# Derek-TH-Wang/quadruped_ctrl

Hardware: AMD Instinct MI355X
Metric: convex-MPC QP solves/sec (horizon=10, 4-leg) (higher is better)
Workload: dtype f64

## Files before the change

quadruped_ctrl_amd/csrc/qmpc_kernels.hip:

```cpp
#include <hip/hip_runtime.h>
#include <stdint.h>

#include <type_traits>

#include "qmpc_device.h"
#include "qmpc_cmd.h"
#include "qmpc_wave.h"

namespace {

__device__ __forceinline__ void fmac16_rowbcast(double (&a)[16], double c, double u) {
  asm volatile(
      "s_nop 1\n\t"
      "v_fmac_f64_dpp %0, %16, %17 row_newbcast:0 row_mask:0xf bank_mask:0xf\n\t"
      "v_fmac_f64_dpp %1, %16, %17 row_newbcast:1 row_mask:0xf bank_mask:0xf\n\t"
      "v_fmac_f64_dpp %2, %16, %17 row_newbcast:2 row_mask:0xf bank_mask:0xf\n\t"
      "v_fmac_f64_dpp %3, %16, %17 row_newbcast:3 row_mask:0xf bank_mask:0xf\n\t"
      "v_fmac_f64_dpp %4, %16, %17 row_newbcast:4 row_mask:0xf bank_mask:0xf\n\t"
      "v_fmac_f64_dpp %5, %16, %17 row_newbcast:5 row_mask:0xf bank_mask:0xf\n\t"
      "v_fmac_f64_dpp %6, %16, %17 row_newbcast:6 row_mask:0xf bank_mask:0xf\n\t"
      "v_fmac_f64_dpp %7, %16, %17 row_newbcast:7 row_mask:0xf bank_mask:0xf\n\t"
      "v_fmac_f64_dpp %8, %16, %17 row_newbcast:8 row_mask:0xf bank_mask:0xf\n\t"
      "v_fmac_f64_dpp %9, %16, %17 row_newbcast:9 row_mask:0xf bank_mask:0xf\n\t"
      "v_fmac_f64_dpp %10, %16, %17 row_newbcast:10 row_mask:0xf bank_mask:0xf\n\t"
// ... 175 lines not shown
    set0 = (unsigned)__builtin_amdgcn_readlane((int)m, k0);
    const unsigned long long ne = ~(__ballot(m == set0 && lane < h) >> k0);
    run = ne ? __builtin_ctzll(ne) : 64;
    run = run < h - k0 ? run : h - k0;
  }
  const int k = (lane < 3) ? lane : (lane < 6 ? lane - 3 : 0);
  const bool rot = lane < 3, row = lane < 6;
  const float* q = P.q + (size_t)i * 4;
  const float* tr = P.traj + (size_t)i * 12 * h;
  const float T = (float)h * (float)P.dt;
  const float qw = q[0], qx = q[1], qy = q[2], qz = q[3];
  const float ang = (k == 0) ? 2.f * (qw * qx + qy * qz) : (k == 1 ? 2.f * (qw * qy - qz * qx) : P.yaw[i]);
  const float x0 = rot ? ang : P.p[(size_t)i * 3 + k];
  const float xd = rot ? P.w[(size_t)i * 3 + k] : P.v[(size_t)i * 3 + k];
  const float e = (x0 - tr[(rot ? 0 : 3) + k]) + T * (xd - tr[(rot ? 6 : 9) + k]);
  const float wk = P.weights[(size_t)i * P.weights_stride + (rot ? 0 : 3) + k];
  const float ialpha = 1.f / (P.alpha[(size_t)i * P.alpha_stride] + 1e-30f);
  const float t_acc = wk * __builtin_fabsf(e), t_dem = __builtin_sqrtf(wk * ialpha) * __builtin_fabsf(e);
  float acc = 0.f, wsum = 1e-30f, dem = 0.f;
#pragma unroll
  for (int l = 0; l < 6; ++l) {
    acc += __builtin_bit_cast(float, __builtin_amdgcn_readlane(__builtin_bit_cast(int, t_acc), l));
    wsum += __builtin_bit_cast(float, __builtin_amdgcn_readlane(__builtin_bit_cast(int, wk), l));
    dem += __builtin_bit_cast(float, __builtin_amdgcn_readlane(__builtin_bit_cast(int, t_dem), l));
  }
  float score = acc / wsum * (float)first3;
  const float demand = dem * (float)first3 / ((float)P.mass * __builtin_fabsf((float)P.gravity) + 1e-30f);
  float pattern = 0.f;
  if (set0 != 0u) {
    float c3[3] = {0.f, 0.f, 0.f};
#pragma unroll
    for (int ax = 0; ax < 3; ++ax)
#pragma unroll
      for (int f = 0; f < 4; ++f) {
        const float rv = __builtin_bit_cast(float, __builtin_amdgcn_readlane(__builtin_bit_cast(int, rraw), 4 * ax + f));
        c3[ax] += ((set0 >> f) & 1u) ? rv : 0.f;
      }
    const float inv = 1.f / (float)__builtin_popcount(set0);
    const float cx = c3[0] * inv, cy = c3[1] * inv, cz = __builtin_fabsf(c3[2] * inv);
    const float sat = __builtin_sqrtf(cx * cx + cy * cy) * (float)P.mu_inv / (cz > 1e-3f ? cz : 1e-3f);
    const float sa = sat > 0.6f ? (sat < 1.f ? sat : 1.f) : 0.f;
    const float pat = (float)run * sa - 1.5f;
    pattern = pat > 0.f ? pat : 0.f;
    score += 0.15f * pattern;
  }
  return {nst, score, demand, pattern};
}
__device__ __forceinline__ int qmpc_score_level(const float score, const float per, const int levels) {
  int b = (score > 0.f) ? (int)(per * (__log2f(score) + 6.f)) : 0;
  b = b < 0 ? 0 : (b > levels - 1 ? levels - 1 : b);
  return levels - 1 - b;
}

template <int RB>
struct Cfg {
  static constexpr bool C1 = (RB == 1 || RB == 6);
  static constexpr int NP = (RB == 4) ? 96 : (RB == 6 ? 64 : 64 * RB);
  static constexpr int CW = NP / 4;
  static constexpr int NT = 4 * NP;
  static constexpr bool BALANCE = (RB == 4);
  static constexpr int NT_LAUNCH = BALANCE ? 512 : NT;
  static constexpr int RE = (NP + 63) / 64;
  static constexpr int KMAX = C1 ? 64 : 96;
  static constexpr int KW = (KMAX + 63) / 64;
  static constexpr int NS = KMAX * (KMAX + 1) / 2;
  static constexpr int NH = NP * (NP + 1) / 2;
  static constexpr int POOL = (RB == 1) ? 2688 : (RB == 6 ? 1536 : (RB == 2 ? 11400 : (RB == 4 ? 5120 : 1176)));
  static constexpr int NPOOL = POOL;
  static constexpr int KS = C1 ? 32 : (RB == 3 ? 128 : 64);
  static constexpr bool EVENT_ENGINE = true;
  static constexpr bool GLOBAL_EVENTS = (RB == 3);
  static constexpr int KEV_GLOBAL = (RB == 3) ? 160 : 96;
  static constexpr int NHELP = C1 ? 0 : 3;
  static constexpr bool PAIRED = (RB == 2 || RB == 3);
  static constexpr int HELP_MIN_TRIPS = 3;
  static constexpr int HMAX = (RB == 3) ? 36 : 16;
  static constexpr int MIN_WAVES = (RB == 1 || RB == 4) ? 4 : (RB == 6 ? 5 : (RB == 2 ? 2 : 3));
  static constexpr int MIN_WAVES_A = (RB == 2) ? 4 : MIN_WAVES;
};

template <int RB>
struct Smem {
  using C = Cfg<RB>;
  QmpcParams par;
  static constexpr int SLOTS = (RB == 3) ? 144 : 64;
  double fmaxk[SLOTS];
  unsigned char sidx[SLOTS];
  unsigned char kslot[4 * C::HMAX];
  int nst, status;
  int mode;
  int evslot;
  int qnext;
  int prio_rank;
  int bal_simd[8], bal_cu, bal_bit;
  struct Help {
    int cmd;
    int pj1, pj2, neva, nevd, glob;
    double pa1, pa2;
    unsigned long long gptr;
  } hd;
  union U {
    struct AW {
      struct Asm {
        double Mb[4][9];
        double Nb[4][9];
        double W[12];
        static constexpr int TAB = (C::HMAX + 1) * (C::HMAX + 1);
        double ct0[TAB], ct4[TAB];
        double ct1[TAB], ct5[TAB], ct8[TAB];
        double E00[144], E11[144];
        double e[C::HMAX * 12];
        double s[3][C::HMAX * 12];
      } a;
      struct Swp {
        alignas(16) double colbuf[2][2][C::NP + 2];
        double ubuf[2][2][C::NP];
        double g[C::NP];
        double part[4][C::NP];
      } w;
    } aw;
    struct Slv {
      double Hp[C::NH];
      double Sinv[C::NPOOL];
      double D[C::NP];
    } b;
  } u;
};

#ifndef QMPC_DBG_ITER
#define QMPC_DBG_ITER 0
#endif
#define QMPC_TICK1(k)                                                \
  do {                                                               \
    if (dbg_clk && tid == 0 && iters == 0) dbg_clk[(k)] = clock64(); \
  } while (0)
#define QMPC_TICK(k)                                   \
  do {                                                 \
    if (dbg_clk && tid == 0) dbg_clk[(k)] = clock64(); \
  } while (0)

#ifdef QMPC_SWEEP_STAMP
#define QMPC_STEP_TICK(k, dep)                                                                            \
  do {                                                                                                    \
    if (PK.dbg_clk && tid == 0 && k0 == QMPC_SWEEP_STAMP) {                         \
      double dep__ = (dep);                                                                               \
      asm volatile("" ::"v"(dep__));                                                                      \
      PK.dbg_clk[(size_t)(rid + PK.batch) * 16 + (k)] = clock64();                                    \
    }                                                                                                     \
  } while (0)
#else
#define QMPC_STEP_TICK(k, dep) do { } while (0)
#endif

#ifdef QMPC_STOP_AFTER
template <int RB, int NV>
__device__ __forceinline__ void qmpc_census_dump(Smem<RB>& S, const QmpcParams& PK, int rid, int tid, const double (&regs)[NV]) {
  double acc = 0.0;
#pragma unroll
  for (int k = 0; k < NV; ++k) acc += regs[k];
  const volatile double* lds = reinterpret_cast<const volatile double*>(&S);
  for (int k = tid; k < (int)(sizeof(Smem<RB>) / 8); k += Cfg<RB>::NT) acc += lds[k];
  PK.grf[(size_t)rid * 12 + (tid % 12)] = (float)acc;
  if (tid == 0) {
    PK.status[rid] = 0;
    if (PK.iters) PK.iters[rid] = 0;
  }
}
#define QMPC_STOP(k, regs)                                  \
  do {                                                      \
    if constexpr (QMPC_STOP_AFTER == (k)) {                 \
      __syncthreads();                                      \
      qmpc_census_dump<RB>(S, PK, rid, tid, regs);          \
      __syncthreads();                                      \
      return false;                                         \
    }                                                       \
  } while (0)
#else
#define QMPC_STOP(k, regs) do { } while (0)
#endif

template <int RB, bool V5, bool CMD, bool ADMM = false, bool WARM = false, bool PHA = false, bool BIG = false, bool PRIO = false>
__device__ __forceinline__ bool solve_one(const int rid, const int tid, Smem<RB>& S, const QmpcParams& PK) {
  using C = Cfg<RB>;
  constexpr int NP = C::NP, CW = C::CW, NT = C::NT, KMAX = C::KMAX, KW = C::KW, RE = C::RE;
  const QmpcParams& P = S.par;
  const int lane = tid & (WAVE - 1);
  const int i = tid % NP;
  const int c = tid / NP;
  const int h = PK.horizon;
  const int nfs = 4 * h;
  constexpr int HMAX = C::HMAX;
  constexpr int NFG = (4 * HMAX + 63) / 64;
  long long* dbg_clk = PK.dbg_clk ? PK.dbg_clk + (size_t)rid * 16 : nullptr;
  QMPC_TICK(0);
  {
    const double none[1] = {0.0};
    (void)none;
    QMPC_STOP(-1, none);
  }
  __builtin_amdgcn_s_setprio(3);
  bool hard = false;
  int hfloor = 0;
  if (PK.hint_hard > 0) {
    const int32_t* grp = (const int32_t*)__builtin_assume_aligned(PK.hint_iters + (rid & ~15), 64);
    int mine = 0, ge = 0;
#pragma unroll
    for (int k = 0; k < 16; ++k) mine = ((rid & 15) == k) ? grp[k] : mine;
#pragma unroll
    for (int k = 0; k < 16; ++k) ge += (grp[k] >= mine) ? 1 : 0;
    mine = __builtin_amdgcn_readfirstlane(mine);
    ge = __builtin_amdgcn_readfirstlane(ge);
    const int top = __builtin_amdgcn_readfirstlane(*PK.hint_max_r);
    hard = mine >= PK.hint_hard && 5 * mine >= 3 * top && ge <= 2;
    hfloor = hard ? 3 : ((mine >= PK.hint_hard && 5 * mine >= 2 * top && ge <= 4) ? 2 : 0);
  }

  unsigned long long prio_mine = 0ull;
  unsigned long long* prio_word = nullptr;
  auto& Aa = S.u.aw.a;
  auto& Sw = S.u.aw.w;
  const int eidx0 = (tid + NT / 2) % NT;
  const bool e_thr = eidx0 < 12 * h;
  const int ek = eidx0 / 12, erow = eidx0 - 12 * ek;
  const int mt = tid % 36, mb = mt / 9, ml = (mt % 9) / 3, max_ = mt % 3;
  const int hs = h + 1, hh = hs * hs;
  constexpr bool cmdm = CMD;
  static_assert(sizeof(QmpcParams) % 4 == 0 && sizeof(QmpcParams) / 4 <= 256, "parameter block copy");
  uint32_t g_par = 0;
  if (tid < (int)(sizeof(QmpcParams) / 4)) g_par = reinterpret_cast<const uint32_t*>(&PK)[tid];
  float g_yaw = cmdm ? PK.c_rpy[(size_t)rid * 3 + 2] : PK.yaw[rid];
  float g_xdrag = cmdm ? PK.c_xci[rid] : PK.x_drag[(size_t)rid * PK.x_drag_stride];
  float c_p0 = 0.f, c_p1 = 0.f, c_p2 = 0.f;
  QmpcTrajGen tg;
  if (cmdm) {
    const float* pos = PK.c_position + (size_t)rid * 3;
    c_p0 = pos[0];
    c_p1 = pos[1];
    c_p2 = pos[2];
    const bool stand = PK.c_gait_type && PK.c_gait_type[rid] == 4;
    float vw0, vw1;
    qmpc_cmd_vdes_world(PK.c_r_body + (size_t)rid * 9, PK.c_vel_des[(size_t)rid * 3 + 0], PK.c_vel_des[(size_t)rid * 3 + 1],
                        PK.c_omni_mode, vw0, vw1);
    qmpc_cmd_traj_gen(tg, stand, stand ? PK.c_stand_traj + (size_t)rid * 6 : nullptr,
                      PK.c_rp_des ? PK.c_rp_des + (size_t)rid * 2 : nullptr, PK.c_rpy_comp + (size_t)rid * 2,
                      PK.c_yaw_des_true[rid], PK.c_wpd[(size_t)rid * 2 + 0], PK.c_wpd[(size_t)rid * 2 + 1], c_p0, c_p1,
                      PK.c_body_height, PK.c_vel_des[(size_t)rid * 3 + 2], vw0, vw1, (float)PK.dt);
  }
  auto gait_at = [&](int fs) __attribute__((always_inline)) {
    if (cmdm) {
      const int leg = fs & 3;
      return (unsigned char)qmpc_cmd_gait_bit(fs >> 2, PK.c_gait_iteration[rid], PK.c_gait_offsets[(size_t)rid * 4 + leg],
                                              PK.c_gait_durations[(size_t)rid * 4 + leg], h);
    }
    return (unsigned char)PK.gait[(size_t)rid * nfs + fs];
  };
  unsigned char g_gait = 0;
  unsigned char g_gaitx[NFG > 1 ? NFG - 1 : 1] = {};
  if (tid < nfs) g_gait = gait_at(tid);
  if constexpr (NFG > 1) {
    if (tid < WAVE) {
#pragma unroll
      for (int g = 1; g < NFG; ++g)
        if (tid + 64 * g < nfs) g_gaitx[g - 1] = gait_at(tid + 64 * g);
    }
  }
  float g_r0 = 0.f, g_r1 = 0.f, g_r2 = 0.f;
  if (tid < 72) {
    if (cmdm) {
      const float* pf = PK.c_p_foot + (size_t)rid * 12 + 3 * mb;
      g_r0 = qmpc_cmd_foot_offset(pf[0], c_p0);
      g_r1 = qmpc_cmd_foot_offset(pf[1], c_p1);
      g_r2 = qmpc_cmd_foot_offset(pf[2], c_p2);
    } else {
      const float* r = PK.r + (size_t)rid * 12;
      g_r0 = r[0 * 4 + mb];
      g_r1 = r[1 * 4 + mb];
      g_r2 = r[2 * 4 + mb];
    }
  }
  float g_q[4] = {1.f, 0.f, 0.f, 0.f}, g_w[3] = {0.f, 0.f, 0.f}, g_v[3] = {0.f, 0.f, 0.f};
  float g_p = 0.f, g_traj = 0.f, g_wt = 0.f;
  if (e_thr) {
    const float* q = (cmdm ? PK.c_orientation : PK.q) + (size_t)rid * 4;
    const float* om = (cmdm ? PK.c_omega_world : PK.w) + (size_t)rid * 3;
    const float* v = (cmdm ? PK.c_v_world : PK.v) + (size_t)rid * 3;
#pragma unroll
    for (int k = 0; k < 4; ++k) g_q[k] = q[k];
#pragma unroll
    for (int k = 0; k < 3; ++k) {
      g_w[k] = om[k];
      g_v[k] = v[k];
    }
    if (cmdm) {
      if (erow >= 3 && erow < 6) g_p = (erow == 3) ? c_p0 : (erow == 4 ? c_p1 : c_p2);
      g_traj = qmpc_cmd_traj_value(tg, ek, erow);
      g_wt = qmpc_cmd_weight(erow);
    } else {
      if (erow >= 3 && erow < 6) g_p = PK.p[(size_t)rid * 3 + (erow - 3)];
      g_traj = PK.traj[(size_t)rid * 12 * h + eidx0];
      g_wt = PK.weights[(size_t)rid * PK.weights_stride + erow];
    }
  }
  float g_w12 = 0.f;
  if (tid >= 96 && tid < 96 + 12)
    g_w12 = cmdm ? qmpc_cmd_weight(tid - 96) : PK.weights[(size_t)rid * PK.weights_stride + (tid - 96)];
  float g_alpha = cmdm ? 4e-5f : PK.alpha[(size_t)rid * PK.alpha_stride];
  double g_ct0 = 0.0, g_ct4 = 0.0, g_ct1 = 0.0, g_ct5 = 0.0, g_ct8 = 0.0;
  constexpr bool TAB2 = (HMAX + 1) * (HMAX + 1) > NT;
  double g2_ct0 = 0.0, g2_ct4 = 0.0, g2_ct1 = 0.0, g2_ct5 = 0.0, g2_ct8 = 0.0;
  if constexpr (TAB2) {
    if (tid + NT < hh) {
      g2_ct0 = PK.ctab[tid + NT];
      g2_ct4 = PK.ctab[4 * hh + tid + NT];
      g2_ct1 = PK.ctab[1 * hh + tid + NT];
      g2_ct5 = PK.ctab[5 * hh + tid + NT];
      g2_ct8 = PK.ctab[8 * hh + tid + NT];
    }
  }
  if (tid < hh) {
    g_ct0 = PK.ctab[tid];
    g_ct4 = PK.ctab[4 * hh + tid];
    g_ct1 = PK.ctab[1 * hh + tid];
    g_ct5 = PK.ctab[5 * hh + tid];
    g_ct8 = PK.ctab[8 * hh + tid];
  }
  if constexpr (PRIO && !CMD && !ADMM && !BIG && !PHA) {
    if (PK.prio_cu && (tid >> 6) == 1) {
      const QmpcKeys kk = qmpc_robot_keys_wave(PK, rid, lane);
      if (tid == 127) {
        unsigned hwid, xcc;
        asm volatile("s_getreg_b32 %0, hwreg(HW_REG_HW_ID)" : "=s"(hwid));
        asm volatile("s_getreg_b32 %0, hwreg(HW_REG_XCC_ID)" : "=s"(xcc));
        prio_word = PK.prio_cu + (((xcc & 7u) << 8) | ((hwid >> 8) & 0xffu));
        if (kk.demand >= 12.f || kk.pattern > 0.5f) {
          const int pb = qmpc_score_level(kk.score, 6.f, 64);
          prio_mine = ((unsigned long long)PK.prio_tag << 32) | ((unsigned long long)(63 - pb) << 24) | (unsigned)(rid & 0xffffff);
          __hip_atomic_fetch_max(prio_word, prio_mine, __ATOMIC_RELAXED, __HIP_MEMORY_SCOPE_AGENT);
        }
      }
    }
  }
  {
    int gg = g_gait;
    asm volatile("" : "+v"(g_par), "+v"(g_yaw), "+v"(g_xdrag), "+v"(g_alpha), "+v"(gg), "+v"(g_r0), "+v"(g_r1),
                 "+v"(g_r2), "+v"(g_q[0]), "+v"(g_q[1]), "+v"(g_q[2]), "+v"(g_q[3]), "+v"(g_w[0]), "+v"(g_w[1]),
                 "+v"(g_w[2]), "+v"(g_v[0]), "+v"(g_v[1]), "+v"(g_v[2]), "+v"(g_p), "+v"(g_traj), "+v"(g_wt),
                 "+v"(g_w12), "+v"(g_ct0), "+v"(g_ct4), "+v"(g_ct1), "+v"(g_ct5), "+v"(g_ct8));
    g_gait = (unsigned char)gg;
    if constexpr (TAB2) asm volatile("" : "+v"(g2_ct0), "+v"(g2_ct4), "+v"(g2_ct1), "+v"(g2_ct5), "+v"(g2_ct8));
  }
  if (tid < (int)(sizeof(QmpcParams) / 4)) reinterpret_cast<uint32_t*>(&S.par)[tid] = g_par;
  const double x_drag = (double)g_xdrag;
  const bool drag = (x_drag != 0.0);

  if (dbg_clk && tid == 0) {
    float sink = g_yaw + g_traj + (float)g_gait + (float)g_ct0;
    asm volatile("" ::"v"(sink));
    dbg_clk[11] = clock64();
  }
  if (tid < WAVE) {
    int base = 0;
#pragma unroll
    for (int g = 0; g < NFG; ++g) {
      const int fs = tid + 64 * g;
      const float fm = (float)(g == 0 ? g_gait : g_gaitx[g > 0 ? g - 1 : 0]) * (float)PK.f_max;
      const bool st = fs < nfs && (((ADMM || BIG) && PK.admm_mode == 1) ? true : !(fm < 0.01f && fm > -.01f));
      const unsigned long long mask = __ballot(st);
      const int pos = base + __popcll(mask & ((1ull << tid) - 1ull));
      if (st && pos < Smem<RB>::SLOTS) {
        S.sidx[pos] = (unsigned char)fs;
        S.fmaxk[pos] = (double)fm;
      }
      if (fs < 4 * HMAX) S.kslot[fs] = (st && pos < Smem<RB>::SLOTS) ? (unsigned char)pos : (unsigned char)0xff;
      base += __popcll(mask);
    }
    if (tid == 0) {
      S.nst = base;
      S.status = 0;
    }
  }
  if (PK.soln)
    for (int k = tid; k < 12 * h; k += NT) PK.soln[(size_t)rid * 12 * h + k] = 0.0;

  const double inv_m = PK.inv_mass;
  {
    float syf, cyf;
    sincosf(g_yaw, &syf, &cyf);
    const double cy = cyf, sy = syf;
    if (PK.dbg_aux && tid == 0) {
      PK.dbg_aux[(size_t)rid * 8 + 0] = cy;
      PK.dbg_aux[(size_t)rid * 8 + 1] = sy;
    }
    if (tid < 72) {
      const int b = mb, l = ml, ax = max_;
      const double ix = PK.inv_ibody[0], iy = PK.inv_ibody[1], iz = PK.inv_ibody[2];
      const double en = __builtin_fma(cy, cy, sy * sy) - 1.0;
      const double isc = 1.0 - 2.0 * en + 3.0 * en * en;
      const double I00 = (cy * cy * ix + sy * sy * iy) * isc, I01 = (cy * sy * (ix - iy)) * isc,
                   I11 = (sy * sy * ix + cy * cy * iy) * isc;
      const double rx = g_r0, ry = g_r1, rz = g_r2;
      const double cm0 = (ax == 0) ? 0.0 : (ax == 1 ? -rz : ry);
      const double cm1 = (ax == 0) ? rz : (ax == 1 ? 0.0 : -rx);
      const double cm2 = (ax == 0) ? -ry : (ax == 1 ? rx : 0.0);
      const double m0 = I00 * cm0 + I01 * cm1;
      const double m1 = I01 * cm0 + I11 * cm1;
      const double m2 = iz * cm2;
      if (tid < 36) {
        Aa.Mb[b][3 * l + ax] = (l == 0) ? m0 : (l == 1 ? m1 : m2);
      } else {
        Aa.Nb[b][3 * l + ax] = (l == 0) ? (cy * m0 + sy * m1) : (l == 1 ? (-sy * m0 + cy * m1) : m2);
      }
    } else if (tid >= 96 && tid < 96 + 12) {
      Aa.W[tid - 96] = (double)g_w12;
    }
    if (e_thr) {
      const int row = erow;
      const double t = (double)(ek + 1) * PK.dt;
      double val;
      if (row < 3) {
#pragma clang fp contract(off)
        const float w = g_q[0], x = g_q[1], y = g_q[2], z = g_q[3];
        const float a_num = (row == 0) ? 2.f * (y * z + w * x) : 2.f * (x * y + w * z);
        const float a_den = (row == 0) ? (w * w - x * x - y * y + z * z) : (w * w + x * x - y * y - z * z);
        float ang = atan2f(a_num, a_den);
        if (row == 1) {
          double asd = -2. * (double)(x * z - w * y);
          if (!(asd < .99999)) asd = .99999;
          ang = asinf((float)asd);
        }
        const double o0 = g_w[0], o1 = g_w[1], o2 = g_w[2];
        const double rate = (row == 0) ? (cy * o0 + sy * o1) : (row == 1 ? (-sy * o0 + cy * o1) : o2);
        if (PK.dbg_aux && ek == 0) PK.dbg_aux[(size_t)rid * 8 + 2 + row] = (double)ang;
        val = (double)ang + rate * t;
      } else if (row < 6) {
        val = (double)g_p + (double)(row == 3 ? g_v[0] : (row == 4 ? g_v[1] : g_v[2])) * t;
        if (row == 5) {
          val += (PK.model == 1) ? 0.5 * PK.gravity * (t * t - t * PK.dt)
                                 : 0.5 * (PK.gravity + x_drag * (double)g_v[0]) * t * t;
        }
      } else if (row < 9) {
        val = (double)(row == 6 ? g_w[0] : (row == 7 ? g_w[1] : g_w[2]));
      } else {
        val = (double)(row == 9 ? g_v[0] : (row == 10 ? g_v[1] : g_v[2]));
        if (row == 11) val += (PK.gravity + x_drag * (double)g_v[0]) * t;
      }
      Aa.e[eidx0] = (double)g_wt * (val - (double)g_traj);
    }
    if (tid < hh) {
      Aa.ct0[tid] = g_ct0;
      Aa.ct4[tid] = g_ct4;
      if (drag) {
        Aa.ct1[tid] = g_ct1;
        Aa.ct5[tid] = g_ct5;
        Aa.ct8[tid] = g_ct8;
      }
    }
    if constexpr (TAB2) {
      if (tid + NT < hh) {
        Aa.ct0[tid + NT] = g2_ct0;
        Aa.ct4[tid + NT] = g2_ct4;
        if (drag) {
          Aa.ct1[tid + NT] = g2_ct1;
          Aa.ct5[tid + NT] = g2_ct5;
          Aa.ct8[tid + NT] = g2_ct8;
        }
      }
    }
  }
  if (dbg_clk && tid == 0) dbg_clk[12] = clock64();
  __syncthreads();
  QMPC_TICK(1);
  if constexpr (PRIO && !CMD && !ADMM && !BIG && !PHA) {
    if (PK.prio_cu && tid == 127) {
      const unsigned long long pv = __hip_atomic_load(prio_word, __ATOMIC_RELAXED, __HIP_MEMORY_SCOPE_AGENT);
      S.prio_rank = (prio_mine != 0ull && pv == prio_mine) ? 0 : ((unsigned)(pv >> 32) == PK.prio_tag ? 1 : 2);
    }
  }
  {
    const double keep0[2] = {(double)g_alpha, x_drag};
    (void)keep0;
    QMPC_STOP(0, keep0);
  }
  if (PK.hint_hard > 0 && !hard) __builtin_amdgcn_s_setprio(2);
  const int nst = S.nst;
  const int n = 3 * nst;
  auto cmd_finish_state = [&]() __attribute__((always_inline)) {
    const float* pos = P.c_position + (size_t)rid * 3;
    if (!(P.c_gait_type && P.c_gait_type[rid] == 4)) {
      P.c_wpd[(size_t)rid * 2 + 0] = qmpc_cmd_clamp(P.c_wpd[(size_t)rid * 2 + 0], pos[0]);
      P.c_wpd[(size_t)rid * 2 + 1] = qmpc_cmd_clamp(P.c_wpd[(size_t)rid * 2 + 1], pos[1]);
    }
    P.c_xci[rid] = qmpc_cmd_xci_next(P.c_xci[rid], pos[2], P.c_body_height, (float)P.dt, P.c_v_world[(size_t)rid * 3 + 0]);
  };
  auto cmd_finish_forces = [&](const float* fb, int l12) __attribute__((always_inline)) {
    const int leg = l12 / 3, ii = l12 - 3 * leg;
    P.f_ff[(size_t)rid * 12 + l12] =
        qmpc_cmd_f2b(P.c_r_body + (size_t)rid * 9 + 3 * ii, fb[3 * leg], fb[3 * leg + 1], fb[3 * leg + 2]);
  };
  static_assert(!BIG || (RB == 3 && PHA && !ADMM && !WARM), "large-problem producer: an instantiation of the 192-row class");
  if (nst == 0 || n > (BIG ? 3 * Smem<RB>::SLOTS : NP)) {
    if (nst == 0) {
      if (tid < 12) P.grf[(size_t)rid * 12 + tid] = 0.f;
      if (cmdm && P.f_ff && tid < 12) P.f_ff[(size_t)rid * 12 + tid] = 0.f;
      if (tid == 0) {
        P.status[rid] = 0;
        if (P.iters) P.iters[rid] = 0;
        if (cmdm) cmd_finish_state();
      }
      if (WARM && P.ws && tid < QMPC_WS_STRIDE) P.ws[(size_t)rid * QMPC_WS_STRIDE + tid] = -1;
    } else if (P.next_list) {
      if (tid == 0) {
        const int slot = atomicAdd(P.next_count, 1);
        if (slot < P.batch) {
          P.next_list[slot] = rid;
        } else {
          P.status[rid] = QMPC_DEV_ST_WS_FULL;
          if (P.iters) P.iters[rid] = 0;
          for (int k = 0; k < 12; ++k) P.grf[(size_t)rid * 12 + k] = 0.f;
        }
      }
    } else {
      if (tid < 12) P.grf[(size_t)rid * 12 + tid] = 0.f;
      if (cmdm && P.f_ff && tid < 12) P.f_ff[(size_t)rid * 12 + tid] = 0.f;
      if (tid == 0) {
        P.status[rid] = QMPC_DEV_ST_WS_FULL;
        if (P.iters) P.iters[rid] = 0;
        if (cmdm) cmd_finish_state();
      }
    }
    __syncthreads();
    return false;
  }
  const double alpha = (double)g_alpha;
  if constexpr (PHA) {
    if (tid == 0) S.evslot = P.wk_base + atomicAdd(P.wk_count, 1);
  }
  if (tid < 144) {
    const int u = tid / 12, v = tid - 12 * u;
    const int bu = u / 3, au = u - 3 * bu, bv = v / 3, av = v - 3 * bv;
    double e00 = 0.0, e11 = 0.0;
#pragma unroll
    for (int l = 0; l < 3; ++l) {
      e00 += Aa.W[6 + l] * (Aa.Mb[bu][3 * l + au] * Aa.Mb[bv][3 * l + av]);
      e11 += Aa.W[l] * (Aa.Nb[bu][3 * l + au] * Aa.Nb[bv][3 * l + av]);
    }
    if (au == av) {
      e00 += Aa.W[9 + au] * (inv_m * inv_m);
      e11 += Aa.W[3 + au] * (inv_m * inv_m);
      if (drag && au == 0) e11 += Aa.W[11] * ((x_drag * inv_m) * (x_drag * inv_m));
    }
    Aa.E00[tid] = e00;
    Aa.E11[tid] = e11;
  }
  if constexpr (HMAX <= 16) {
    if (tid >= 64 && tid < 256) {
      const int row = (tid - 64) >> 4, st = tid & 15;
      auto shl = [](double x, auto nc) __attribute__((always_inline)) {
        constexpr int N = decltype(nc)::value;
        const unsigned long long b = (unsigned long long)__double_as_longlong(x);
        const unsigned lo = (unsigned)__builtin_amdgcn_mov_dpp((int)(unsigned)b, 0x100 + N, 0xf, 0xf, true);
        const unsigned hi = (unsigned)__builtin_amdgcn_mov_dpp((int)(unsigned)(b >> 32), 0x100 + N, 0xf, 0xf, true);
        return __longlong_as_double((long long)(((unsigned long long)hi << 32) | lo));
      };
      auto suffix = [&](double x) __attribute__((always_inline)) {
        x += shl(x, std::integral_constant<int, 1>{});
        x += shl(x, std::integral_constant<int, 2>{});
        x += shl(x, std::integral_constant<int, 4>{});
        x += shl(x, std::integral_constant<int, 8>{});
        return x;
      };
      const double e = (st < h) ? Aa.e[st * 12 + row] : 0.0;
      const double S0 = suffix(e);
      const double S1 = suffix(shl(S0, std::integral_constant<int, 1>{}));
      const double T2 = suffix(shl(S1, std::integral_constant<int, 1>{}));
      const double S2 = 2.0 * T2 + S1;
      const double dt1 = P.dt, dt2 = dt1 * dt1, dt3 = dt2 * dt1;
      if (st < h) {
        Aa.s[0][st * 12 + row] = dt1 * S0;
        Aa.s[1][st * 12 + row] = (P.model == 1) ? dt2 * S1 : dt2 * S1 + (0.5 * dt2) * S0;
        Aa.s[2][st * 12 + row] = (0.5 * dt3) * (S2 + S1) + (dt3 / 6.0) * S0;
      }
    }
  } else if (tid >= 192 && tid < 204) {
    const int row = tid - 192;
    double ek[HMAX];
#pragma unroll
    for (int k = 0; k < HMAX; ++k) ek[k] = Aa.e[(k < h ? k : 0) * 12 + row];
    const double dt1 = P.dt, dt2 = dt1 * dt1, dt3 = dt2 * dt1;
    double S0 = 0.0, S1 = 0.0, S2 = 0.0;
#pragma unroll
    for (int st = HMAX - 1; st >= 0; --st) {
      if (st < h) {
        S2 = S2 + 2.0 * S1 + S0;
        S1 = S1 + S0;
        S0 = S0 + ek[st];
        Aa.s[0][st * 12 + row] = dt1 * S0;
        Aa.s[1][st * 12 + row] = (P.model == 1) ? dt2 * S1 : dt2 * S1 + (0.5 * dt2) * S0;
        Aa.s[2][st * 12 + row] = (0.5 * dt3) * (S2 + S1) + (dt3 / 6.0) * S0;
      }
    }
  }
  __syncthreads();
  QMPC_TICK(2);
  if constexpr (PRIO && !CMD && !ADMM && !BIG && !PHA) {
    if (PK.prio_cu && __builtin_amdgcn_readfirstlane(S.prio_rank) == 1) __builtin_amdgcn_s_setprio(2);
  }
  {
    const double keep1[2] = {alpha, x_drag};
    (void)keep1;
    QMPC_STOP(1, keep1);
  }
  if constexpr (PHA) {
    if (S.evslot - P.wk_base >= P.wk_cap) {
      if (tid < 12) P.grf[(size_t)rid * 12 + tid] = 0.f;
      if (cmdm && P.f_ff && tid < 12) P.f_ff[(size_t)rid * 12 + tid] = 0.f;
      if (tid == 0) {
        P.status[rid] = QMPC_DEV_ST_WS_FULL;
        if (P.iters) P.iters[rid] = 0;
        if (cmdm) cmd_finish_state();
      }
      __syncthreads();
      return false;
    }
  }

#ifdef QMPC_BIG_STAMP
#define QMPC_BIG_TICK(k) do { if (dbg_clk && tid == 0) dbg_clk[(k)] = clock64(); } while (0)
#define QMPC_BIG_STEP_TICK(k) do { if (dbg_clk && tid == 0 && k0 == NB * QMPC_BIG_STAMP) dbg_clk[(k)] = clock64(); } while (0)
#else
#define QMPC_BIG_TICK(k) do { } while (0)
#define QMPC_BIG_STEP_TICK(k) do { } while (0)
#endif
  if constexpr (BIG) {
    constexpr int LDB = QMPC_BIG_LD, NB = 16, PD = NB + 1, NMAX = 3 * Smem<RB>::SLOTS;
    const int item = S.evslot;
    GlobalF64* const A = (GlobalF64*)P.wk_hinv + (size_t)item * ((size_t)LDB * LDB);
    auto ldA = [&](int r, int cidx) __attribute__((always_inline)) {
      return __hip_atomic_load(A + (size_t)r * LDB + cidx, __ATOMIC_RELAXED, __HIP_MEMORY_SCOPE_WORKGROUP);
    };
    const int wv = tid >> 6;
    constexpr int NWV = NT / 64;
    const double dm2 = x_drag * inv_m * inv_m;

    QMPC_BIG_TICK(8);
    double gmine = 0.0;
    if (tid < n) {
      const int ki = S.sidx[tid / 3], ax = tid % 3;
      const int st = ki >> 2, b = ki & 3;
      const double* s0 = &Aa.s[0][st * 12];
      const double* s1 = &Aa.s[1][st * 12];
      double acc = s0[9 + ax] * inv_m + s1[3 + ax] * inv_m;
#pragma unroll
      for (int l = 0; l < 3; ++l) acc += Aa.Mb[b][3 * l + ax] * s0[6 + l] + Aa.Nb[b][3 * l + ax] * s1[l];
      if (drag && ax == 0) acc += (x_drag * inv_m) * (s1[11] + Aa.s[2][st * 12 + 5]);
      gmine = 2.0 * acc;
    }
    {
      const double w11 = Aa.W[11] * dm2, w5 = Aa.W[5] * dm2, w5x = Aa.W[5] * (x_drag * dm2);
      for (int r = wv; r < n; r += NWV) {
        const int ki = S.sidx[r / 3], ai = r % 3, si = ki >> 2, u = 3 * (ki & 3) + ai;
        for (int j = lane; j < n; j += 64) {
          const int kj = S.sidx[j / 3], cax = j % 3, sj = kj >> 2;
          const int cidx = si * hs + sj, tidx = sj * hs + si, eidx = u * 12 + 3 * (kj & 3) + cax;
          double v = Aa.ct0[cidx] * Aa.E00[eidx] + Aa.ct4[cidx] * Aa.E11[eidx];
          if (drag) {
            double add = 0.0;
            if (ai == 2 && cax == 0) add = Aa.ct1[cidx] * w11 + Aa.ct5[cidx] * w5;
            if (ai == 0 && cax == 2) add = Aa.ct1[tidx] * w11 + Aa.ct5[tidx] * w5;
            if (ai == 0 && cax == 0) add = Aa.ct8[cidx] * w5x;
            v += add;
          }
          double hv = 2.0 * (v + ((r == j) ? alpha : 0.0));
          if (P.admm_mode != 0 && r == j) {
            const double fk = S.fmaxk[r / 3];
            const double rho4 = (__builtin_fabs(fk) < 1e-10) ? P.admm_rho * 1e3 : (fk > 1e10 ? 1e-6 : P.admm_rho);
            hv += P.admm_sigma + ((ai < 2) ? 2.0 * 1e-6 * P.mu_inv * P.mu_inv : 4.0 * 1e-6 + rho4);
          }
          A[(size_t)r * LDB + j] = hv;
        }
      }
    }
    __syncthreads();
    QMPC_BIG_TICK(9);
    double* const Cp = reinterpret_cast<double*>(&S.u);
    double* const Fp = Cp + NMAX * PD;
    double* const Pm = Fp + NMAX * PD;
    double* const Qm = Pm + NB * PD;
    double* const Rm = Qm + NB * PD;
    double* const gl = Rm + NB * PD;
    constexpr int NTLMAX = (NMAX + 15) / 16, TLW = (NTLMAX * (NTLMAX + 1) / 2 + NWV - 1) / NWV;
    unsigned short* const tl = reinterpret_cast<unsigned short*>(gl + NMAX);
    static_assert(sizeof(double) * (2 * NMAX * PD + 3 * NB * PD + NMAX) + 2 * NWV * TLW <= sizeof(S.u), "scratch of the block sweep");
    if (tid < NMAX) gl[tid] = gmine;
    {
      const int ntl0 = (n + 15) >> 4, ntiles = ntl0 * (ntl0 + 1) / 2;
      for (int pq = tid; pq < ntiles; pq += NT) {
        int ti0 = (int)((__builtin_sqrtf(8.f * (float)pq + 1.f) - 1.f) * 0.5f);
        while (ti0 * (ti0 + 1) / 2 > pq) --ti0;
        while ((ti0 + 1) * (ti0 + 2) / 2 <= pq) ++ti0;
        tl[(pq % NWV) * TLW + pq / NWV] = (unsigned short)((ti0 << 8) | (pq - ti0 * (ti0 + 1) / 2));
      }
    }
    bool bad = false;
#pragma unroll 1
    for (int k0 = 0; k0 < n; k0 += NB) {
      const int bsz = (n - k0 < NB) ? n - k0 : NB;
      QMPC_BIG_STEP_TICK(0);
      if (tid < NB * NB) {
        const int pi = tid / NB, pj = tid % NB;
        Pm[pi * PD + pj] = (pi < bsz && pj < bsz) ? ldA(k0 + (pi > pj ? pi : pj), k0 + (pi > pj ? pj : pi)) : ((pi == pj) ? 1.0 : 0.0);
      }
      for (int e = tid; e < n * NB; e += NT) {
        const int r = e / NB, kk = e % NB, cc = k0 + kk;
        Cp[r * PD + kk] = (kk < bsz) ? (r >= cc ? ldA(r, cc) : ldA(cc, r)) : 0.0;
      }
      __syncthreads();
      QMPC_BIG_STEP_TICK(1);
      if (wv == 0) {
        const int i16 = lane & 15;
        double pr[NB];
#pragma unroll
        for (int j = 0; j < NB; ++j) pr[j] = Pm[i16 * PD + j];
        StaticFor<0, NB>::run([&](auto ppc) __attribute__((always_inline)) {
          constexpr int pp = decltype(ppc)::value;
          double d = 0.0;
          fmac_rowbcast<pp>(d, pr[pp], 1.0);
          bad |= !(d > 0.0);
          double rl = __builtin_amdgcn_rsq(d);
          double e = __builtin_fma(-d * rl, rl, 1.0);
          rl = __builtin_fma(0.5 * rl, e, rl);
          e = __builtin_fma(-d * rl, rl, 1.0);
          rl = __builtin_fma(0.5 * rl, e, rl);
          const double l = pr[pp] * rl;
          pr[pp] = (i16 == pp) ? rl : l;
          const double cl = (i16 > pp) ? l : 0.0;
          fmac16_rowbcast(pr, cl, -cl);
        });
        if (lane < NB) {
#pragma unroll
          for (int j = 0; j < NB; ++j) Pm[lane * PD + j] = pr[j];
        }
        __builtin_amdgcn_wave_barrier();
        QMPC_BIG_STEP_TICK(7);
        {
          double x[NB];
          StaticFor<0, NB>::run([&](auto ic) __attribute__((always_inline)) {
            constexpr int i2 = decltype(ic)::value;
            double acc = (i2 == i16) ? 1.0 : 0.0;
            StaticFor<0, i2>::run([&](auto mc) __attribute__((always_inline)) {
              constexpr int m = decltype(mc)::value;
              acc = __builtin_fma(-Pm[i2 * PD + m], x[m], acc);
            });
            x[i2] = acc * Pm[i2 * PD + i2];
            if (lane < NB) Qm[i2 * PD + lane] = x[i2];
// ... 195 lines not shown
      for (int sl = tid; sl < nst; sl += 64) {
        const double x0 = Fp[3 * sl], x1 = Fp[3 * sl + 1], x2 = Fp[3 * sl + 2];
        const double fx = P.mu_inv * x0, fy = P.mu_inv * x1, nt = -P.tol, ifr = P.inv_fr_norm;
        viol += ((fx + x2) * ifr < nt) + ((x2 - fx) * ifr < nt) + ((fy + x2) * ifr < nt) + ((x2 - fy) * ifr < nt) +
                (S.fmaxk[sl] - x2 < nt);
      }
#pragma unroll
      for (int sft = 1; sft < 64; sft <<= 1) viol += __shfl_xor(viol, sft);
      if (tid == 0) {
        const int lvl = viol >> 4;
        const int b = QMPC_ORDER_BUCKETS - 1 - (lvl < QMPC_ORDER_BUCKETS - 1 ? lvl : QMPC_ORDER_BUCKETS - 1);
        const int pos = atomicAdd(P.wk_bucket + b, 1);
        P.wk_order[(size_t)b * P.wk_cap + P.wk_base + pos] = item;
      }
    }
    __syncthreads();
    return false;
  }

  if (tid < NP) {
    double gv = 0.0;
    if (tid < n) {
      const int ki = S.sidx[tid / 3], ax = tid % 3;
      const int st = ki >> 2, b = ki & 3;
      const double* s0 = &Aa.s[0][st * 12];
      const double* s1 = &Aa.s[1][st * 12];
      double acc = s0[9 + ax] * inv_m + s1[3 + ax] * inv_m;
#pragma unroll
      for (int l = 0; l < 3; ++l)
        acc += Aa.Mb[b][3 * l + ax] * s0[6 + l] + Aa.Nb[b][3 * l + ax] * s1[l];
      if (drag && ax == 0) acc += (x_drag * inv_m) * (s1[11] + Aa.s[2][st * 12 + 5]);
      gv = 2.0 * acc;
    }
    Sw.g[tid] = gv;
  }

  if (dbg_clk && tid == 0) dbg_clk[13] = clock64();
  double a[CW];
  {
    const bool rowok = i < n;
    const int ki = rowok ? (int)S.sidx[(i / 3) & 63] : 0;
    const int ai = rowok ? i % 3 : 0;
    const int si = rowok ? (ki >> 2) : h;
    const int u = 3 * (ki & 3) + ai;
    const double dm2 = x_drag * inv_m * inv_m;
    double admm_diag = 0.0;
    if constexpr (ADMM) {
      const double fk = rowok ? S.fmaxk[(i / 3) & 63] : 1.0;
      const double rho4 = (__builtin_fabs(fk) < 1e-10) ? P.admm_rho * 1e3 : (fk > 1e10 ? 1e-6 : P.admm_rho);
      admm_diag = P.admm_sigma + ((ai < 2) ? 2.0 * 1e-6 * P.mu_inv * P.mu_inv : 4.0 * 1e-6 + rho4);
    }
    constexpr int NSL = CW / 3 + 2;
    const int cslot0 = (c * CW) / 3, cax0 = (c * CW) % 3;
    constexpr bool PACK = (RB == 3);
    int kjs[PACK ? (NSL + 3) / 4 : NSL];
    if constexpr (PACK) {
#pragma unroll
      for (int q4 = 0; q4 < (NSL + 3) / 4; ++q4) {
        unsigned w = 0;
#pragma unroll
        for (int b = 0; b < 4; ++b) {
          const int sl = cslot0 + 4 * q4 + b;
          const unsigned kv = S.sidx[sl < 63 ? sl : 63];
          w |= ((sl < nst) ? kv : (unsigned)(4 * h)) << (8 * b);
        }
        kjs[q4] = (int)w;
      }
    } else {
#pragma unroll
      for (int q = 0; q < NSL; ++q) {
        const int sl = cslot0 + q;
        const int kv = (int)S.sidx[sl < 63 ? sl : 63];
        kjs[q] = (sl < nst) ? kv : 4 * h;
      }
    }
    auto kj_at = [&](int q) __attribute__((always_inline)) {
      if constexpr (PACK) return (int)(((unsigned)kjs[q >> 2] >> (8 * (q & 3))) & 0xffu);
      else return kjs[q];
    };
    auto fill = [&](auto cax0c) __attribute__((always_inline)) {
      constexpr int CAX0 = decltype(cax0c)::value;
      if constexpr (RB == 3) {
#pragma unroll
        for (int jj = 0; jj < CW; ++jj) {
          const int kj = kj_at((CAX0 + jj) / 3), cax = (CAX0 + jj) % 3;
          const int cidx = si * hs + (kj >> 2), eidx = u * 12 + 3 * (kj & 3) + cax;
          a[jj] = Aa.ct0[cidx] * Aa.E00[eidx] + Aa.ct4[cidx] * Aa.E11[eidx];
          if ((jj & 1) == 1) __builtin_amdgcn_sched_barrier(0);
        }
      } else {
        constexpr int NS = (CAX0 + CW - 1) / 3 + 1;
        double t0[NS], t4[NS];
#pragma unroll
        for (int q = 0; q < NS; ++q) {
          const int cidx = si * hs + (kj_at(q) >> 2);
          t0[q] = Aa.ct0[cidx];
          t4[q] = Aa.ct4[cidx];
        }
#pragma unroll
        for (int jj = 0; jj < CW; ++jj) {
          constexpr int dummy = 0;
          (void)dummy;
          const int q = (CAX0 + jj) / 3, cax = (CAX0 + jj) % 3;
          const int eidx = u * 12 + 3 * (kj_at(q) & 3) + cax;
          a[jj] = t0[q] * Aa.E00[eidx] + t4[q] * Aa.E11[eidx];
          if ((jj & 3) == 3) __builtin_amdgcn_sched_barrier(0);
        }
      }
      if ((RB == 2 || RB == 3) ? __builtin_expect(drag, false) : drag) {
        const double w11 = Aa.W[11] * dm2, w5 = Aa.W[5] * dm2, w5x = Aa.W[5] * (x_drag * dm2);
#pragma unroll
        for (int jj = 0; jj < CW; ++jj) {
          const int kj = kj_at((CAX0 + jj) / 3), cax = (CAX0 + jj) % 3;
          const int sj = kj >> 2, cidx = si * hs + sj, tidx = sj * hs + si;
          double add = 0.0;
          if (ai == 2 && cax == 0) add = Aa.ct1[cidx] * w11 + Aa.ct5[cidx] * w5;
          if (ai == 0 && cax == 2) add = Aa.ct1[tidx] * w11 + Aa.ct5[tidx] * w5;
          if (ai == 0 && cax == 0) add = Aa.ct8[cidx] * w5x;
          a[jj] += add;
          if (RB == 3 || (jj & 3) == 3) __builtin_amdgcn_sched_barrier(0);
        }
      }
    };
    if (cax0 == 0) fill(std::integral_constant<int, 0>{});
    else if (cax0 == 1) fill(std::integral_constant<int, 1>{});
    else fill(std::integral_constant<int, 2>{});
    if constexpr (RB != 3) {
      const int dd = i - c * CW;
      const double dval = rowok ? alpha : 0.5;
      const double dadm = (ADMM && rowok) ? admm_diag : 0.0;
#pragma unroll
      for (int jj = 0; jj < CW; ++jj) {
        double v = 2.0 * (a[jj] + ((dd == jj) ? dval : 0.0));
        if constexpr (ADMM) v += (dd == jj) ? dadm : 0.0;
        a[jj] = v;
      }
    } else {
#pragma unroll
      for (int jj = 0; jj < CW; ++jj) {
        const int j = c * CW + jj;
        double v = 2.0 * (a[jj] + ((i == j) ? alpha : 0.0));
        if constexpr (ADMM) v += (i == j) ? admm_diag : 0.0;
        a[jj] = (rowok && j < n) ? v : ((i == j) ? 1.0 : 0.0);
      }
    }
  }
  if (P.dbg_H) {
    double* Hd = P.dbg_H + (size_t)rid * QMPC_DBG_LD * QMPC_DBG_LD;
#pragma unroll
    for (int jj = 0; jj < CW; ++jj) Hd[(size_t)i * QMPC_DBG_LD + c * CW + jj] = a[jj];
    if (tid < NP) P.dbg_g[(size_t)rid * QMPC_DBG_LD + tid] = Sw.g[tid];
  }
  QMPC_TICK(3);
  QMPC_STOP(2, a);

  bool notpd = false;
  bool staged = PK.hint_hard > 0;
  if constexpr (PRIO && !CMD && !ADMM && !BIG && !PHA) {
    if (PK.prio_cu) {
      const int rank = __builtin_amdgcn_readfirstlane(S.prio_rank);
      if (QMPC_DBG_ITER == 0 && dbg_clk && tid == 0) dbg_clk[14] = rank;
      hard = rank == 0;
      hfloor = hard ? 3 : 0;
      staged = rank < 2;
    }
  }
  if constexpr (C::C1) {
    double pd0, pe, pd1, pdet, px, pc0, pc1, pm0, pm1;
    auto prod_read = [&](double c0n, double c1n, int k0n) __attribute__((always_inline)) {
      pd0 = readlane_f64(c0n, k0n);
      pe = readlane_f64(c0n, k0n + 1);
      pd1 = readlane_f64(c1n, k0n + 1);
      pm0 = (i == k0n) ? 1.0 : 0.0;
      pm1 = (i == k0n + 1) ? 1.0 : 0.0;
      pc0 = c0n - pm0;
      pc1 = c1n - pm1;
    };
    auto prod_det = [&]() __attribute__((always_inline)) {
      pdet = __builtin_fma(pd0, pd1, -pe * pe);
      notpd |= !(pd0 > 0.0) | !(pdet > 0.0);
    };
    auto prod_rcp = [&]() __attribute__((always_inline)) { px = __builtin_amdgcn_rcp(pdet); };
    auto prod_newton = [&]() __attribute__((always_inline)) {
      const double e1 = __builtin_fma(-pdet, px, 1.0);
      px = __builtin_fma(px, e1, px);
    };
    double pnf0, pnf1;
    double pt0, pt1;
    auto prod_adj = [&]() __attribute__((always_inline)) {
      pt0 = __builtin_fma(pe, pc1, -pd1 * pc0);
      pt1 = __builtin_fma(pe, pc0, -pd0 * pc1);
    };
    auto prod_fg = [&]() __attribute__((always_inline)) {
      pnf0 = pt0 * px;
      pnf1 = pt1 * px;
    };
    auto prod_store = [&](int mn) __attribute__((always_inline)) {
      Sw.colbuf[mn & 1][0][i] = pc0;
      Sw.colbuf[mn & 1][1][i] = pc1;
      Sw.ubuf[mn & 1][0][i] = pnf0;
      Sw.ubuf[mn & 1][1][i] = pnf1;
    };
    if (c == 0) {
      prod_read(a[0], a[1], 0);
      a[0] = __builtin_fma(-2.0, pm0, a[0]);
      a[1] = __builtin_fma(-2.0, pm1, a[1]);
      prod_det();
      prod_rcp();
      prod_adj();
      prod_newton();
      prod_newton();
      prod_fg();
      prod_store(0);
    }
    __syncthreads();
#define QMPC_PIN __builtin_amdgcn_sched_barrier(0)
#pragma unroll 1
    for (int kb = 0; kb < 4; ++kb) {
      if (hard || (kb == 0 && !staged)) __builtin_amdgcn_s_setprio(3);
      else if (kb <= 1 || hfloor >= 2) __builtin_amdgcn_s_setprio(2);
      else if (kb == 2) __builtin_amdgcn_s_setprio(1);
      else __builtin_amdgcn_s_setprio(0);
      StaticFor<0, CW / 2>::run([&](auto pc) __attribute__((always_inline)) {
        constexpr int r0 = 2 * decltype(pc)::value;
        constexpr int rn0 = (r0 + 2 < CW) ? r0 + 2 : 0, rn1 = rn0 + 1;
        constexpr int G0 = 4 * (rn0 / 4), G1 = (G0 + 4) % 16, G2 = (G0 + 8) % 16, G3 = (G0 + 12) % 16;
        const int k0 = kb * CW + r0;
        if (k0 < n) {
          const int m = k0 >> 1;
          const double cv0 = Sw.colbuf[m & 1][0][c * CW + (lane & 15)];
          const double cv1 = Sw.colbuf[m & 1][1][c * CW + (lane & 15)];
          const double nu0 = Sw.ubuf[m & 1][0][i], nu1 = Sw.ubuf[m & 1][1][i];
          const int kbn = (r0 + 2 < CW) ? kb : kb + 1;
          if (k0 + 2 < n && c == kbn) {
            fmac4_rowbcast<G0>(a, cv0, nu0);
            fmac4_rowbcast<G0>(a, cv1, nu1);
            QMPC_PIN;
            prod_read(a[rn0], a[rn1], k0 + 2);
            a[rn0] = __builtin_fma(-2.0, pm0, a[rn0]);
            a[rn1] = __builtin_fma(-2.0, pm1, a[rn1]);
            QMPC_PIN;
            fmac4_rowbcast<G1>(a, cv0, nu0);
            QMPC_PIN;
            prod_det();
            prod_rcp();
            prod_adj();
            QMPC_PIN;
            fmac4_rowbcast<G1>(a, cv1, nu1);
            QMPC_PIN;
            prod_newton();
            QMPC_PIN;
            fmac4_rowbcast<G2>(a, cv0, nu0);
            QMPC_PIN;
            prod_newton();
            QMPC_PIN;
            fmac4_rowbcast<G2>(a, cv1, nu1);
            QMPC_PIN;
            prod_fg();
            QMPC_PIN;
            fmac4_rowbcast<G3>(a, cv0, nu0);
            QMPC_PIN;
            prod_store(m + 1);
            QMPC_PIN;
            fmac4_rowbcast<G3>(a, cv1, nu1);
          } else if (c * CW < n) {
            fmac16_rowbcast(a, cv0, nu0);
            fmac16_rowbcast(a, cv1, nu1);
          }
          __syncthreads();
        }
      });
    }
#undef QMPC_PIN
  } else {
    auto lane_next = [](double x) __attribute__((always_inline)) {
      const unsigned long long b = (unsigned long long)__double_as_longlong(x);
      const unsigned lo = (unsigned)__builtin_amdgcn_mov_dpp((int)(unsigned)b, 0x101, 0xf, 0xf, true);
      const unsigned hi = (unsigned)__builtin_amdgcn_mov_dpp((int)(unsigned)(b >> 32), 0x101, 0xf, 0xf, true);
      return __longlong_as_double((long long)(((unsigned long long)hi << 32) | lo));
    };
    auto publish_pinv = [&](double d0, double e, double d1p, int par) __attribute__((always_inline)) {
      const double det = __builtin_fma(d0, d1p, -e * e);
      const double idet = fast_rcp(det);
      double* pv = Sw.ubuf[par][0];
      st2(pv, d1p * idet, e * idet);
      st2(pv + 2, d0 * idet, (d0 < det) ? d0 : det);
    };
    if (c == 0) {
      Sw.colbuf[0][0][i] = a[0];
      Sw.colbuf[0][1][i] = a[1];
      const double e_n = lane_next(a[0]), d1_n = lane_next(a[1]);
      if (i == 0) {
        publish_pinv(a[0], e_n, d1_n, 0);
        Sw.colbuf[0][0][i] = a[0] - 1.0;
        a[0] -= 2.0;
      }
      if (i == 1) {
        Sw.colbuf[0][1][i] = a[1] - 1.0;
        a[1] -= 2.0;
      }
    }
    __syncthreads();
#pragma unroll 1
    for (int kb = 0; kb < 4; ++kb) {
      if (hard || (kb == 0 && !staged)) __builtin_amdgcn_s_setprio(3);
      else if (kb <= 1 || hfloor >= 2) __builtin_amdgcn_s_setprio(2);
// ... 1867 lines not shown
```

Measured before the change: 27.81 million.

## Rebalance setup work across waves and defer priority-rank readback past second barrier

```diff
diff --git a/quadruped_ctrl_amd/csrc/qmpc_kernels.hip b/quadruped_ctrl_amd/csrc/qmpc_kernels.hip
--- a/quadruped_ctrl_amd/csrc/qmpc_kernels.hip
+++ b/quadruped_ctrl_amd/csrc/qmpc_kernels.hip
@@ -351,6 +351,15 @@
 #define QMPC_STEP_TICK(k, dep) do { } while (0)
 #endif
 
+#ifdef QMPC_FIXED_STAMP
+#define QMPC_WAVE_TICK(k)                                                                                   \
+  do {                                                                                                      \
+    if (PK.dbg_clk && lane == 0 && tid < 256) PK.dbg_clk[(size_t)(rid + PK.batch) * 16 + (tid >> 6) * 4 + (k)] = clock64(); \
+  } while (0)
+#else
+#define QMPC_WAVE_TICK(k) do { } while (0)
+#endif
+
 #ifdef QMPC_STOP_AFTER
 template <int RB, int NV>
 __device__ __forceinline__ void qmpc_census_dump(Smem<RB>& S, const QmpcParams& PK, int rid, int tid, const double (&regs)[NV]) {
@@ -464,7 +473,7 @@
     }
   }
   float g_r0 = 0.f, g_r1 = 0.f, g_r2 = 0.f;
-  if (tid < 72) {
+  if (tid < 36) {
     if (cmdm) {
       const float* pf = PK.c_p_foot + (size_t)rid * 12 + 3 * mb;
       g_r0 = qmpc_cmd_foot_offset(pf[0], c_p0);
@@ -501,8 +510,8 @@
     }
   }
   float g_w12 = 0.f;
-  if (tid >= 96 && tid < 96 + 12)
-    g_w12 = cmdm ? qmpc_cmd_weight(tid - 96) : PK.weights[(size_t)rid * PK.weights_stride + (tid - 96)];
+  const int w12 = tid - (NT - 12);
+  if (w12 >= 0) g_w12 = cmdm ? qmpc_cmd_weight(w12) : PK.weights[(size_t)rid * PK.weights_stride + w12];
   float g_alpha = cmdm ? 4e-5f : PK.alpha[(size_t)rid * PK.alpha_stride];
   double g_ct0 = 0.0, g_ct4 = 0.0, g_ct1 = 0.0, g_ct5 = 0.0, g_ct8 = 0.0;
   constexpr bool TAB2 = (HMAX + 1) * (HMAX + 1) > NT;
@@ -516,12 +525,13 @@
       g2_ct8 = PK.ctab[8 * hh + tid + NT];
     }
   }
-  if (tid < hh) {
-    g_ct0 = PK.ctab[tid];
-    g_ct4 = PK.ctab[4 * hh + tid];
-    g_ct1 = PK.ctab[1 * hh + tid];
-    g_ct5 = PK.ctab[5 * hh + tid];
-    g_ct8 = PK.ctab[8 * hh + tid];
+  const int tix = NT - 1 - tid;
+  if (tix < hh) {
+    g_ct0 = PK.ctab[tix];
+    g_ct4 = PK.ctab[4 * hh + tix];
+    g_ct1 = PK.ctab[1 * hh + tix];
+    g_ct5 = PK.ctab[5 * hh + tix];
+    g_ct8 = PK.ctab[8 * hh + tix];
   }
   if constexpr (PRIO && !CMD && !ADMM && !BIG && !PHA) {
     if (PK.prio_cu && (tid >> 6) == 1) {
@@ -536,6 +546,7 @@
           prio_mine = ((unsigned long long)PK.prio_tag << 32) | ((unsigned long long)(63 - pb) << 24) | (unsigned)(rid & 0xffffff);
           __hip_atomic_fetch_max(prio_word, prio_mine, __ATOMIC_RELAXED, __HIP_MEMORY_SCOPE_AGENT);
         }
+        S.prio_rank = (prio_mine != 0ull) ? (int)(unsigned)(prio_mine & 0xffffffffull) : -1;
       }
     }
   }
@@ -557,6 +568,13 @@
     asm volatile("" ::"v"(sink));
     dbg_clk[11] = clock64();
   }
+#ifdef QMPC_FIXED_STAMP
+  {
+    float sink = g_yaw + g_traj + (float)g_gait + (float)g_ct0 + g_q[0] + g_r0 + g_w12;
+    asm volatile("" ::"v"(sink));
+    QMPC_WAVE_TICK(0);
+  }
+#endif
   if (tid < WAVE) {
     int base = 0;
 #pragma unroll
@@ -583,14 +601,14 @@
 
   const double inv_m = PK.inv_mass;
   {
-    float syf, cyf;
-    sincosf(g_yaw, &syf, &cyf);
+    float syf = 0.f, cyf = 1.f;
+    if (__ballot(tid < 36 || e_thr) != 0ull) sincosf(g_yaw, &syf, &cyf);
     const double cy = cyf, sy = syf;
     if (PK.dbg_aux && tid == 0) {
       PK.dbg_aux[(size_t)rid * 8 + 0] = cy;
       PK.dbg_aux[(size_t)rid * 8 + 1] = sy;
     }
-    if (tid < 72) {
+    if (tid < 36) {
       const int b = mb, l = ml, ax = max_;
       const double ix = PK.inv_ibody[0], iy = PK.inv_ibody[1], iz = PK.inv_ibody[2];
       const double en = __builtin_fma(cy, cy, sy * sy) - 1.0;
@@ -604,14 +622,10 @@
       const double m0 = I00 * cm0 + I01 * cm1;
       const double m1 = I01 * cm0 + I11 * cm1;
       const double m2 = iz * cm2;
-      if (tid < 36) {
-        Aa.Mb[b][3 * l + ax] = (l == 0) ? m0 : (l == 1 ? m1 : m2);
-      } else {
-        Aa.Nb[b][3 * l + ax] = (l == 0) ? (cy * m0 + sy * m1) : (l == 1 ? (-sy * m0 + cy * m1) : m2);
-      }
-    } else if (tid >= 96 && tid < 96 + 12) {
-      Aa.W[tid - 96] = (double)g_w12;
-    }
+      Aa.Mb[b][3 * l + ax] = (l == 0) ? m0 : (l == 1 ? m1 : m2);
+      Aa.Nb[b][3 * l + ax] = (l == 0) ? (cy * m0 + sy * m1) : (l == 1 ? (-sy * m0 + cy * m1) : m2);
+    }
+    if (w12 >= 0) Aa.W[w12] = (double)g_w12;
     if (e_thr) {
       const int row = erow;
       const double t = (double)(ek + 1) * PK.dt;
@@ -645,13 +659,13 @@
       }
       Aa.e[eidx0] = (double)g_wt * (val - (double)g_traj);
     }
-    if (tid < hh) {
-      Aa.ct0[tid] = g_ct0;
-      Aa.ct4[tid] = g_ct4;
+    if (tix < hh) {
+      Aa.ct0[tix] = g_ct0;
+      Aa.ct4[tix] = g_ct4;
       if (drag) {
-        Aa.ct1[tid] = g_ct1;
-        Aa.ct5[tid] = g_ct5;
-        Aa.ct8[tid] = g_ct8;
+        Aa.ct1[tix] = g_ct1;
+        Aa.ct5[tix] = g_ct5;
+        Aa.ct8[tix] = g_ct8;
       }
     }
     if constexpr (TAB2) {
@@ -667,14 +681,9 @@
     }
   }
   if (dbg_clk && tid == 0) dbg_clk[12] = clock64();
+  QMPC_WAVE_TICK(1);
   __syncthreads();
   QMPC_TICK(1);
-  if constexpr (PRIO && !CMD && !ADMM && !BIG && !PHA) {
-    if (PK.prio_cu && tid == 127) {
-      const unsigned long long pv = __hip_atomic_load(prio_word, __ATOMIC_RELAXED, __HIP_MEMORY_SCOPE_AGENT);
-      S.prio_rank = (prio_mine != 0ull && pv == prio_mine) ? 0 : ((unsigned)(pv >> 32) == PK.prio_tag ? 1 : 2);
-    }
-  }
   {
     const double keep0[2] = {(double)g_alpha, x_drag};
     (void)keep0;
@@ -799,6 +808,19 @@
       }
     }
   }
+  if constexpr (PRIO && !CMD && !ADMM && !BIG && !PHA) {
+    if (P.prio_cu && tid == NT - 1) {
+      unsigned hwid, xcc;
+      asm volatile("s_getreg_b32 %0, hwreg(HW_REG_HW_ID)" : "=s"(hwid));
+      asm volatile("s_getreg_b32 %0, hwreg(HW_REG_XCC_ID)" : "=s"(xcc));
+      const unsigned long long* wd = P.prio_cu + (((xcc & 7u) << 8) | ((hwid >> 8) & 0xffu));
+      const int mine32 = S.prio_rank;
+      const unsigned long long pv = __hip_atomic_load(wd, __ATOMIC_RELAXED, __HIP_MEMORY_SCOPE_AGENT);
+      const bool call = (unsigned)(pv >> 32) == P.prio_tag;
+      S.prio_rank = (call && mine32 >= 0 && (unsigned)pv == (unsigned)mine32) ? 0 : (call ? 1 : 2);
+    }
+  }
+  QMPC_WAVE_TICK(2);
   __syncthreads();
   QMPC_TICK(2);
   if constexpr (PRIO && !CMD && !ADMM && !BIG && !PHA) {
@@ -1300,6 +1322,10 @@
     if (tid < NP) P.dbg_g[(size_t)rid * QMPC_DBG_LD + tid] = Sw.g[tid];
   }
   QMPC_TICK(3);
+#ifdef QMPC_FIXED_STAMP
+  asm volatile("" ::"v"(a[0]), "v"(a[CW - 1]));
+  QMPC_WAVE_TICK(3);
+#endif
   QMPC_STOP(2, a);
 
   bool notpd = false;
```

Measured after the change: 28.32 million (median of 6 runs). 1.8% higher.
